# sonbui25/Multimodal-Aspect-Category-Sentiment-Analysis

Measured on AMD Instinct MI355X. Metric: train samples/sec (fwd+bwd+step) FCMF seq128x36ROI, higher is better.
Workload: dtype bf16; 1 GPU; FCMF-base fine-tune step, BASELINE configs[1]: batch 64 reviews x 6 aspects per GPU, seq 128, 7 images x (49 patches + 36 ROIs), precomputed ResNet-152 features, dropout 0.1, clip 1.0 + 4-group AdamW + linear schedule; global_batch=64, per_gpu_batch=64, seq_len=128, parallelism=dp1, sample_unit=1 review = 6 aspect forwards

## Files before the change

multimodal-aspect-category-sentiment-analysis_amd/csrc/attn_mfma.hip:

```cpp
#include "attn_tiles.h"
#include <cstdlib>


template <int NKT>
__device__ __forceinline__ void attn_mfma_fwd_tile(const AttnMfmaParams& P, int g, int h, int q0, int lane, const bf16x8 (&qf)[2][2],
                                                   const char* Ks, const char* Vs, const float* mask_lds = nullptr) {
  constexpr int NKF = 8 * NKT;
  const float* mrow = P.mask ? P.mask + (int64_t)g * P.Tk : nullptr;
  int nvalid = P.Tk;
  if (mask_lds || mrow) {
    int last = -1;
#pragma unroll
    for (int i = 0; i < 2 * NKT; ++i) {
      const int key = 64 * i + lane;
      const bool live = key < P.Tk && (mask_lds ? mask_lds[key] : mrow[key]) > -1e30f;
      const unsigned long long b = __ballot(live);
      if (b) last = 64 * i + 63 - __builtin_clzll(b);
    }
    nvalid = last >= 0 ? last + 1 : P.Tk;
  }
  f32x4 sc[NKF][2];
#pragma unroll
  for (int kf = 0; kf < NKF; ++kf)
#pragma unroll
    for (int f = 0; f < 2; ++f) sc[kf][f] = f32x4{0.f, 0.f, 0.f, 0.f};
#pragma unroll
  for (int s = 0; s < 2; ++s)
#pragma unroll
    for (int kf = 0; kf < NKF; ++kf) {
      if (16 * kf >= nvalid) continue;
      const bf16x8 ka = frag_row64(Ks, 16 * kf, s, lane);
#pragma unroll
      for (int f = 0; f < 2; ++f) sc[kf][f] = __builtin_amdgcn_mfma_f32_16x16x32_bf16(ka, qf[f][s], sc[kf][f], 0, 0, 0);
    }
  const float inv_keep = P.p > 0.f ? 1.0f / (1.0f - P.p) : 1.0f;
#pragma unroll
  for (int f = 0; f < 2; ++f) {
    const int q = q0 + 16 * f + (lane & 15);
    float m = -INFINITY;
#pragma unroll
    for (int kf = 0; kf < NKF; ++kf) {
      if (16 * kf >= nvalid) continue;
#pragma unroll
      for (int r = 0; r < 4; ++r) {
        const int key = 16 * kf + 4 * (lane >> 4) + r;
        float s = -INFINITY;
        if (key < P.Tk) s = sc[kf][f][r] * P.scale + (mask_lds ? mask_lds[key] : (mrow ? mrow[key] : 0.f));
        sc[kf][f][r] = s;
        m = fmaxf(m, s);
      }
    }
    m = fmaxf(m, __shfl_xor(m, 16, 64));
    m = fmaxf(m, __shfl_xor(m, 32, 64));
    float sum = 0.f;
#pragma unroll
    for (int kf = 0; kf < NKF; ++kf) {
      if (16 * kf >= nvalid) continue;
#pragma unroll
      for (int r = 0; r < 4; ++r) {
        const float e = __expf(sc[kf][f][r] - m);
        sc[kf][f][r] = e;
        sum += e;
      }
    }
    sum += __shfl_xor(sum, 16, 64);
    sum += __shfl_xor(sum, 32, 64);
    const float inv = 1.0f / sum;
    if (q < P.Tq && (lane >> 4) == 0 && P.lse) P.lse[((int64_t)g * P.heads + h) * P.Tq + q] = m + __logf(sum);
#pragma unroll
    for (int kf = 0; kf < NKF; ++kf) {
      if (16 * kf >= nvalid) continue;
      float dm[4] = {1.f, 1.f, 1.f, 1.f};
      if (P.p > 0.f)
        dropout_mult4(P.seed, ((uint64_t)g * P.heads + h) * P.Tq * P.Tk + (__umul24((unsigned)q, (unsigned)P.Tk) + (unsigned)(16 * kf + 4 * (lane >> 4))),
                      P.p, inv_keep, dm);
#pragma unroll
      for (int r = 0; r < 4; ++r) sc[kf][f][r] = sc[kf][f][r] * inv * dm[r];
    }
  }
  f32x4 oc[4][2];
#pragma unroll
  for (int df = 0; df < 4; ++df)
#pragma unroll
    for (int f = 0; f < 2; ++f) oc[df][f] = f32x4{0.f, 0.f, 0.f, 0.f};
#pragma unroll
  for (int s = 0; s < 4 * NKT; ++s) {
    if (32 * s >= nvalid) continue;
    bf16x8 pb[2];
#pragma unroll
    for (int f = 0; f < 2; ++f)
#pragma unroll
      for (int r = 0; r < 4; ++r) { pb[f][r] = (bf16_t)sc[2 * s][f][r]; pb[f][4 + r] = (bf16_t)sc[2 * s + 1][f][r]; }
#pragma unroll
    for (int df = 0; df < 4; ++df) {
      const bf16x8 va = frag_tr64p(Vs, 16 * df, s, lane);
#pragma unroll
      for (int f = 0; f < 2; ++f) oc[df][f] = __builtin_amdgcn_mfma_f32_16x16x32_bf16(va, pb[f], oc[df][f], 0, 0, 0);
    }
  }
#pragma unroll
  for (int f = 0; f < 2; ++f) {
    const int q = q0 + 16 * f + (lane & 15);
    if (q < P.Tq) {
      bf16_t* orow = P.out + ((int64_t)g * P.Tq + q) * P.ldo + h * AD + 4 * (lane >> 4);
#pragma unroll
      for (int df = 0; df < 4; ++df) store4(orow + 16 * df, oc[df][f]);
    }
  }
}

template <int NKT>
__device__ __forceinline__ void attn_mfma_fwd_body(const AttnMfmaParams& P) {
  extern __shared__ __attribute__((aligned(16))) char smem[];
  char* Ks = smem;
  char* Vs = smem + NKT * TILE_B;
  const int tid = threadIdx.x, lane = tid & 63, w = tid >> 6;
  const int g = blockIdx.x / P.heads, h = blockIdx.x % P.heads;
  const int q0 = blockIdx.y * AT + w * 32;
  const bf16_t* kbase_p = P.k + (int64_t)g * P.Tk * P.ldk + h * AD;
  const bf16_t* vbase_p = P.v + (int64_t)g * P.Tk * P.ldk + h * AD;
  const TileRegs kt = load_tile(kbase_p, P.ldk, P.Tk, tid);
  const TileRegs vt = load_tile(vbase_p, P.ldk, P.Tk, tid);
  bf16x8 qf[2][2];
  load_q_frags(P, g, h, q0, lane, qf);
  store_tile<false>(Ks, kt, tid);
  store_tile<true>(Vs, vt, tid);
  if constexpr (NKT == 2) {
    const TileRegs kt2 = load_tile(kbase_p + (int64_t)AT * P.ldk, P.ldk, P.Tk - AT, tid);
    const TileRegs vt2 = load_tile(vbase_p + (int64_t)AT * P.ldk, P.ldk, P.Tk - AT, tid);
    store_tile<false>(Ks + TILE_B, kt2, tid);
    store_tile<true>(Vs + TILE_B, vt2, tid);
  }
  __syncthreads();
  attn_mfma_fwd_tile<NKT>(P, g, h, q0, lane, qf, Ks, Vs);
}

__global__ __launch_bounds__(256, 2) void attn_mfma_fwd_persist_kernel(AttnMfmaParams P, int ntiles, int qtiles) {
  extern __shared__ __attribute__((aligned(16))) char smem[];
  const int tid = threadIdx.x, lane = tid & 63, w = tid >> 6;
  auto where = [&](int tile, int& g, int& h, int& q0) {
    const int gh = tile / qtiles;
    g = gh / P.heads; h = gh - g * P.heads; q0 = (tile - gh * qtiles) * AT + w * 32;
  };
  constexpr int BUF = 2 * TILE_B + 512;
  int tile = blockIdx.x;
  if (tile >= ntiles) return;
  int g, h, q0;
  where(tile, g, h, q0);
  bf16x8 qf[2][2];
  auto mask_of = [&](int gg) { return (P.mask && tid < P.Tk) ? P.mask[(int64_t)gg * P.Tk + tid] : 0.f; };
  {
    const TileRegs kt = load_tile(P.k + (int64_t)g * P.Tk * P.ldk + h * AD, P.ldk, P.Tk, tid);
    const TileRegs vt = load_tile(P.v + (int64_t)g * P.Tk * P.ldk + h * AD, P.ldk, P.Tk, tid);
    const float mv = mask_of(g);
    load_q_frags(P, g, h, q0, lane, qf);
    store_tile<false>(smem, kt, tid);
    store_tile<true>(smem + TILE_B, vt, tid);
    if (tid < AT) reinterpret_cast<float*>(smem + 2 * TILE_B)[tid] = mv;
  }
  __syncthreads();
  int cur = 0;
  for (;;) {
    const int nxt = tile + gridDim.x;
    const bool more = nxt < ntiles;
    int g2 = g, h2 = h, q2 = q0;
    TileRegs kt, vt;
    bf16x8 qn[2][2];
    float mv = 0.f;
    if (more) {
      where(nxt, g2, h2, q2);
      kt = load_tile(P.k + (int64_t)g2 * P.Tk * P.ldk + h2 * AD, P.ldk, P.Tk, tid);
      vt = load_tile(P.v + (int64_t)g2 * P.Tk * P.ldk + h2 * AD, P.ldk, P.Tk, tid);
      mv = mask_of(g2);
      load_q_frags(P, g2, h2, q2, lane, qn);
    }
    const char* buf = smem + cur * BUF;
    attn_mfma_fwd_tile<1>(P, g, h, q0, lane, qf, buf, buf + TILE_B, reinterpret_cast<const float*>(buf + 2 * TILE_B));
    if (!more) break;
    cur ^= 1;
    store_tile<false>(smem + cur * BUF, kt, tid);
    store_tile<true>(smem + cur * BUF + TILE_B, vt, tid);
    if (tid < AT) reinterpret_cast<float*>(smem + cur * BUF + 2 * TILE_B)[tid] = mv;
#pragma unroll
    for (int f = 0; f < 2; ++f)
#pragma unroll
      for (int s2 = 0; s2 < 2; ++s2) qf[f][s2] = qn[f][s2];
    g = g2; h = h2; q0 = q2; tile = nxt;
    __syncthreads();
  }
}

__global__ __launch_bounds__(256, 3) void attn_mfma_fwd_kernel(AttnMfmaParams P) { attn_mfma_fwd_body<1>(P); }
__global__ __launch_bounds__(256, 2) void attn_mfma_fwd256_kernel(AttnMfmaParams P) { attn_mfma_fwd_body<2>(P); }

template <int NQT, int NKT>
__device__ __forceinline__ void attn_mfma_bwd_body(const AttnMfmaParams& P) {
  extern __shared__ __attribute__((aligned(16))) char smem[];
  char* Qs = smem;
  char* dOs = Qs + NQT * TILE_B;
  char* Ks = dOs + NQT * TILE_B;
  char* Vs = Ks + NKT * TILE_B;
  char* PdT = Vs + NKT * TILE_B;
  char* dST = PdT + TILE_B / 2;
  const int tid = threadIdx.x, lane = tid & 63, w = tid >> 6;
  const int g = blockIdx.x / P.heads, h = blockIdx.x % P.heads;
  const int64_t qbase = (int64_t)g * P.Tq, kbase = (int64_t)g * P.Tk;
  float dl4[NQT][2][4], lse4[NQT][2][4];
  {
    TileRegs tq[NQT], td[NQT];
#pragma unroll
    for (int qt = 0; qt < NQT; ++qt) {
      tq[qt] = load_tile(P.q + (qbase + qt * AT) * P.ldq + h * AD, P.ldq, P.Tq - qt * AT, tid);
      td[qt] = load_tile(P.dout + (qbase + qt * AT) * P.ldo + h * AD, P.ldo, P.Tq - qt * AT, tid);
    }
    TileRegs tk = load_tile(P.k + kbase * P.ldk + h * AD, P.ldk, P.Tk, tid);
    TileRegs tv = load_tile(P.v + kbase * P.ldk + h * AD, P.ldk, P.Tk, tid);
#pragma unroll
    for (int qt = 0; qt < NQT; ++qt) {
      const int q = qt * AT + 32 * w + (lane >> 1), half = lane & 1;
      float sd = 0.f;
      if (q < P.Tq) {
        const bf16_t* a = P.dout + (qbase + q) * P.ldo + h * AD + 32 * half;
        const bf16_t* b = P.o + (qbase + q) * P.ldo + h * AD + 32 * half;
#pragma unroll
        for (int i = 0; i < 4; ++i) {
          const bf16x8 x = *reinterpret_cast<const bf16x8*>(a + 8 * i);
          const bf16x8 y = *reinterpret_cast<const bf16x8*>(b + 8 * i);
#pragma unroll
          for (int j = 0; j < 8; ++j) sd += (float)x[j] * (float)y[j];
        }
      }
      sd += __shfl_xor(sd, 1, 64);
#pragma unroll
      for (int f = 0; f < 2; ++f)
#pragma unroll
        for (int r = 0; r < 4; ++r) {
          const int ql = 16 * f + 4 * (lane >> 4) + r;
          dl4[qt][f][r] = __shfl(sd, 2 * ql, 64);
          const int q2 = qt * AT + 32 * w + ql;
          lse4[qt][f][r] = q2 < P.Tq ? P.lse[((int64_t)g * P.heads + h) * P.Tq + q2] : 0.f;
        }
    }
#pragma unroll
    for (int qt = 0; qt < NQT; ++qt) {
      store_tile<false>(Qs + qt * TILE_B, tq[qt], tid);
      store_tile<false>(dOs + qt * TILE_B, td[qt], tid);
    }
    store_tile<false>(Ks, tk, tid);
    store_tile<false>(Vs, tv, tid);
    if constexpr (NKT == 2) {
      tk = load_tile(P.k + (kbase + AT) * P.ldk + h * AD, P.ldk, P.Tk - AT, tid);
      tv = load_tile(P.v + (kbase + AT) * P.ldk + h * AD, P.ldk, P.Tk - AT, tid);
      store_tile<false>(Ks + TILE_B, tk, tid);
      store_tile<false>(Vs + TILE_B, tv, tid);
    }
  }
  __syncthreads();

  const float inv_keep = P.p > 0.f ? 1.0f / (1.0f - P.p) : 1.0f;
  const uint64_t drop_base = ((uint64_t)g * P.heads + h) * P.Tq * P.Tk;
  const float* mrow = P.mask ? P.mask + kbase : nullptr;
  float score_scale = P.scale;
  bf16x8 qa[NQT][2][2], da[NQT][2][2], oT[NQT][4], qT[NQT][4];
  f32x4 aQ[NQT][4][2];
#pragma unroll
  for (int qt = 0; qt < NQT; ++qt) {
#pragma unroll
    for (int f = 0; f < 2; ++f)
#pragma unroll
      for (int s = 0; s < 2; ++s) {
        qa[qt][f][s] = frag_row64(Qs + qt * TILE_B, 32 * w + 16 * f, s, lane);
        da[qt][f][s] = frag_row64(dOs + qt * TILE_B, 32 * w + 16 * f, s, lane);
      }
#pragma unroll
    for (int s = 0; s < 4; ++s) {
      oT[qt][s] = frag_tr64(dOs + qt * TILE_B, 16 * w, s, lane);
      qT[qt][s] = frag_tr64(Qs + qt * TILE_B, 16 * w, s, lane);
    }
#pragma unroll
    for (int df = 0; df < 4; ++df)
#pragma unroll
      for (int f = 0; f < 2; ++f) aQ[qt][df][f] = f32x4{0.f, 0.f, 0.f, 0.f};
  }

  const int nchunks_all = (P.Tk + 31) >> 5;
  int nvalid = P.Tk;
  if (mrow) {
    int last = -1;
#pragma unroll
    for (int i = 0; i < 2 * NKT; ++i) {
      const int key = 64 * i + lane;
      const bool live = key < P.Tk && mrow[key] > -1e30f;
      const unsigned long long b = __ballot(live);
      if (b) last = 64 * i + 63 - __builtin_clzll(b);
    }
    nvalid = last >= 0 ? last + 1 : P.Tk;
    if (last < 0) {
      mrow = nullptr;
      score_scale = 0.f;
      const float ltk = __logf((float)P.Tk);
#pragma unroll
      for (int qt = 0; qt < NQT; ++qt)
#pragma unroll
        for (int f = 0; f < 2; ++f)
#pragma unroll
          for (int r = 0; r < 4; ++r) lse4[qt][f][r] = ltk;
    }
  }
  const int nchunks = (nvalid + 31) >> 5;
  const uint64_t pair_base = drop_base >> 1;
  const uint32_t pb_lo = (uint32_t)pair_base, pb_hi = (uint32_t)(pair_base >> 32);
  const bool share_hash = P.p > 0.f && (P.Tk & 1) == 0 && pb_lo <= 0xFFFF0000u;
  const uint32_t hash_k0 = (uint32_t)P.seed ^ ((pb_hi << 7) | (pb_hi >> 25)), hash_s1 = (uint32_t)(P.seed >> 32);
  const uint32_t drop_thr = dropout_threshold(P.p);
  const int odd = lane & 1;
  f32x4 cV = f32x4{0.f, 0.f, 0.f, 0.f}, cK = f32x4{0.f, 0.f, 0.f, 0.f};
  for (int c = 0; c < nchunks; ++c) {
    f32x4 aV[2], aK[2];
#pragma unroll
    for (int kf = 0; kf < 2; ++kf) { aV[kf] = f32x4{0.f, 0.f, 0.f, 0.f}; aK[kf] = f32x4{0.f, 0.f, 0.f, 0.f}; }
#pragma unroll
    for (int qt = 0; qt < NQT; ++qt) {
      f32x4 sS[2][2], sP[2][2];
#pragma unroll
      for (int k4 = 0; k4 < 2; ++k4)
#pragma unroll
        for (int f = 0; f < 2; ++f) { sS[k4][f] = f32x4{0.f, 0.f, 0.f, 0.f}; sP[k4][f] = f32x4{0.f, 0.f, 0.f, 0.f}; }
#pragma unroll
      for (int s = 0; s < 2; ++s)
#pragma unroll
        for (int k4 = 0; k4 < 2; ++k4) {
          const bf16x8 kb = frag_row64(Ks, 32 * c + 16 * k4, s, lane);
          const bf16x8 vb = frag_row64(Vs, 32 * c + 16 * k4, s, lane);
#pragma unroll
          for (int f = 0; f < 2; ++f) {
            sS[k4][f] = __builtin_amdgcn_mfma_f32_16x16x32_bf16(qa[qt][f][s], kb, sS[k4][f], 0, 0, 0);
            sP[k4][f] = __builtin_amdgcn_mfma_f32_16x16x32_bf16(da[qt][f][s], vb, sP[k4][f], 0, 0, 0);
          }
        }
#pragma unroll
      for (int k4 = 0; k4 < 2; ++k4) {
        const int kl = 16 * k4 + (lane & 15), key = 32 * c + kl;
        const float mk = (mrow && key < P.Tk) ? mrow[key] : 0.f;
#pragma unroll
        for (int f = 0; f < 2; ++f) {
          f32x4 pdv, dsv;
          float mult4[4] = {1.0f, 1.0f, 1.0f, 1.0f};
          if (share_hash) {
            const unsigned q0 = qt * AT + 32 * w + 16 * f + 4 * (lane >> 4);
            const uint32_t o0 = pb_lo + __umul24(q0 + 2 * odd, (unsigned)P.Tk >> 1) + ((unsigned)key >> 1);
            const uint32_t hA = fcmf_hash32_rounds(o0 ^ hash_k0, hash_s1);
            const uint32_t hB = fcmf_hash32_rounds((o0 + ((unsigned)P.Tk >> 1)) ^ hash_k0, hash_s1);
            const uint32_t nA = (uint32_t)__builtin_amdgcn_update_dpp(0, (int)hA, 0xB1, 0xf, 0xf, true);
            const uint32_t nB = (uint32_t)__builtin_amdgcn_update_dpp(0, (int)hB, 0xB1, 0xf, 0xf, true);
            const uint32_t hr[4] = {odd ? nA : hA, odd ? nB : hB, odd ? hA : nA, odd ? hB : nB};
#pragma unroll
            for (int r = 0; r < 4; ++r) mult4[r] = ((hr[r] >> (16 * odd)) & 0xFFFFu) >= drop_thr ? inv_keep : 0.f;
          }
#pragma unroll
          for (int r = 0; r < 4; ++r) {
            const int q = qt * AT + 32 * w + 16 * f + 4 * (lane >> 4) + r;
            float pr = 0.f, mult = mult4[r];
            if (key < P.Tk && q < P.Tq) pr = __expf(sS[k4][f][r] * score_scale + mk - lse4[qt][f][r]);
            if (P.p > 0.f && !share_hash) mult = dropout_mult(P.seed, drop_base + (__umul24((unsigned)q, (unsigned)P.Tk) + (unsigned)key), P.p, inv_keep);
            pdv[r] = pr * mult;
            dsv[r] = pr * (sP[k4][f][r] * mult - dl4[qt][f][r]);
          }
          const int ch = 4 * w + 2 * f + (lane >> 5);
          const int o = off128(kl, ch) + ((lane >> 4) & 1) * 8;
          store4(reinterpret_cast<bf16_t*>(PdT + o), pdv);
          store4(reinterpret_cast<bf16_t*>(dST + o), dsv);
        }
      }
      __syncthreads();
      {
        bf16x8 tb[2];
#pragma unroll
        for (int f = 0; f < 2; ++f) tb[f] = frag_tr128(dST, 32 * w + 16 * f, 0, lane);
#pragma unroll
        for (int df = 0; df < 4; ++df) {
          const bf16x8 ka2 = frag_tr64(Ks, 16 * df, c, lane);
#pragma unroll
          for (int f = 0; f < 2; ++f) aQ[qt][df][f] = __builtin_amdgcn_mfma_f32_16x16x32_bf16(ka2, tb[f], aQ[qt][df][f], 0, 0, 0);
        }
      }
#pragma unroll
      for (int s = 0; s < 4; ++s)
#pragma unroll
        for (int kf = 0; kf < 2; ++kf) {
          const bf16x8 pb = frag_row128(PdT, 16 * kf, s, lane);
          const bf16x8 sb = frag_row128(dST, 16 * kf, s, lane);
          aV[kf] = __builtin_amdgcn_mfma_f32_16x16x32_bf16(oT[qt][s], pb, aV[kf], 0, 0, 0);
          aK[kf] = __builtin_amdgcn_mfma_f32_16x16x32_bf16(qT[qt][s], sb, aK[kf], 0, 0, 0);
        }
      __syncthreads();
    }
    const int dcol = h * AD + 16 * w + 4 * (lane >> 4);
    cV += aV[0] + aV[1];
    cK += aK[0] + aK[1];
#pragma unroll
    for (int kf = 0; kf < 2; ++kf) {
      const int key = 32 * c + 16 * kf + (lane & 15);
      if (key < P.Tk) {
        store4(P.dv + (kbase + key) * P.ldk + dcol, aV[kf]);
        f32x4 t = aK[kf];
        t[0] *= P.scale; t[1] *= P.scale; t[2] *= P.scale; t[3] *= P.scale;
        store4(P.dk + (kbase + key) * P.ldk + dcol, t);
      }
    }
  }
  for (int c = nchunks; c < nchunks_all; ++c) {
    const int dcol = h * AD + 16 * w + 4 * (lane >> 4);
#pragma unroll
    for (int kf = 0; kf < 2; ++kf) {
      const int key = 32 * c + 16 * kf + (lane & 15);
      if (key < P.Tk) {
        store4(P.dv + (kbase + key) * P.ldk + dcol, f32x4{0.f, 0.f, 0.f, 0.f});
        store4(P.dk + (kbase + key) * P.ldk + dcol, f32x4{0.f, 0.f, 0.f, 0.f});
      }
    }
  }
#pragma unroll
  for (int qt = 0; qt < NQT; ++qt)
#pragma unroll
    for (int f = 0; f < 2; ++f) {
      const int x = qt * AT + 32 * w + 16 * f + (lane & 15);
      if (x < P.Tq) {
        const int dcol = h * AD + 4 * (lane >> 4);
#pragma unroll
        for (int df = 0; df < 4; ++df) {
          f32x4 t = aQ[qt][df][f];
          t[0] *= P.scale; t[1] *= P.scale; t[2] *= P.scale; t[3] *= P.scale;
          store4(P.dq + (qbase + x) * P.ldq + dcol + 16 * df, t);
        }
      }
    }
  if (P.colsum) {
    const int HD = P.heads * AD;
    float* row = P.colsum + (int64_t)g * 3 * HD + h * AD;
#pragma unroll
    for (int r = 0; r < 4; ++r) { cV[r] = row16_sum(cV[r]); cK[r] = row16_sum(cK[r]); }
    if ((lane & 15) == 0) {
      const int d0 = 16 * w + 4 * (lane >> 4);
#pragma unroll
      for (int r = 0; r < 4; ++r) { row[2 * HD + d0 + r] = cV[r]; row[HD + d0 + r] = cK[r] * P.scale; }
    }
    float* red = reinterpret_cast<float*>(PdT);
#pragma unroll
    for (int df = 0; df < 4; ++df) {
      f32x4 t = f32x4{0.f, 0.f, 0.f, 0.f};
#pragma unroll
      for (int qt = 0; qt < NQT; ++qt)
#pragma unroll
        for (int f = 0; f < 2; ++f) t += aQ[qt][df][f];
#pragma unroll
      for (int r = 0; r < 4; ++r) t[r] = row16_sum(t[r]);
      if ((lane & 15) == 0) {
#pragma unroll
        for (int r = 0; r < 4; ++r) red[w * 64 + 16 * df + 4 * (lane >> 4) + r] = t[r];
      }
    }
    __syncthreads();
    if (tid < 64) row[tid] = (red[tid] + red[64 + tid] + red[128 + tid] + red[192 + tid]) * P.scale;
  }
}

__global__ __launch_bounds__(256, 2) void attn_mfma_bwd_kernel(AttnMfmaParams P) { attn_mfma_bwd_body<1, 1>(P); }
__global__ __launch_bounds__(256, 1) void attn_mfma_bwd256_kernel(AttnMfmaParams P) { attn_mfma_bwd_body<2, 2>(P); }

static bool al16(const void* p) { return (reinterpret_cast<uintptr_t>(p) & 15) == 0; }

extern "C" int fcmf_attn_mfma_fwd(const void* q, const void* k, const void* v, const float* mask, void* out, float* lse,
                                  int G, int heads, int Tq, int Tk, int64_t ldq, int64_t ldk, int64_t ldo, float scale,
                                  float dropout_p, uint64_t seed, void* stream) {
  if (!q || !k || !v || !out || G <= 0 || heads <= 0 || Tq <= 0 || Tk <= 0) return FCMF_ERR_ARG;
  if (Tk > 2 * AT || ldq % 8 || ldk % 8 || ldo % 4 || !al16(q) || !al16(k) || !al16(v) || !al16(out)) return FCMF_ERR_UNSUPPORTED;
  AttnMfmaParams P{};
  P.q = (const bf16_t*)q; P.k = (const bf16_t*)k; P.v = (const bf16_t*)v; P.mask = mask; P.out = (bf16_t*)out; P.lse = lse;
  P.G = G; P.heads = heads; P.Tq = Tq; P.Tk = Tk; P.ldq = ldq; P.ldk = ldk; P.ldo = ldo;
  P.scale = scale; P.p = dropout_p; P.seed = seed;
  const dim3 grid(G * heads, (Tq + AT - 1) / AT);
  if (Tk > AT) {
    const int smem = 4 * TILE_B;
    static bool attr2 = false;
    return fcmf_launch_flagged(&attr2, attn_mfma_fwd256_kernel, grid, dim3(256), smem, reinterpret_cast<hipStream_t>(stream), P);
  }
  const int ntiles = (int)(grid.x * grid.y);
  static const bool no_persist = getenv("FCMF_ATTN_NO_PERSIST") != nullptr;
  if (ntiles >= 4 * 512 && !no_persist) {
    const int smem = 2 * (2 * TILE_B + 512);
    static bool attr3 = false;
    return fcmf_launch_flagged(&attr3, attn_mfma_fwd_persist_kernel, dim3(512), dim3(256), smem, reinterpret_cast<hipStream_t>(stream), P, ntiles, (int)grid.y);
  }
  const int smem = 2 * TILE_B;
  static bool attr = false;
  return fcmf_launch_flagged(&attr, attn_mfma_fwd_kernel, grid, dim3(256), smem, reinterpret_cast<hipStream_t>(stream), P);
}

extern "C" int fcmf_attn_mfma_bwd(const void* q, const void* k, const void* v, const float* mask, const void* out,
                                  const void* dout, const float* lse, void* dq, void* dk, void* dv, int G, int heads,
                                  int Tq, int Tk, int64_t ldq, int64_t ldk, int64_t ldo, float scale, float dropout_p,
                                  uint64_t seed, float* colsum, void* stream) {
  if (!q || !k || !v || !out || !dout || !lse || !dq || !dk || !dv || G <= 0 || heads <= 0 || Tq <= 0 || Tk <= 0) return FCMF_ERR_ARG;
  if (Tk > 2 * AT || Tq > 2 * AT || ldq % 8 || ldk % 8 || ldo % 8 || !al16(q) || !al16(k) || !al16(v) || !al16(out) || !al16(dout) ||
      !al16(dq) || !al16(dk) || !al16(dv))
    return FCMF_ERR_UNSUPPORTED;
  AttnMfmaParams P{};
  P.q = (const bf16_t*)q; P.k = (const bf16_t*)k; P.v = (const bf16_t*)v; P.mask = mask; P.o = (const bf16_t*)out;
  P.dout = (const bf16_t*)dout; P.lse = const_cast<float*>(lse); P.dq = (bf16_t*)dq; P.dk = (bf16_t*)dk; P.dv = (bf16_t*)dv;
  P.G = G; P.heads = heads; P.Tq = Tq; P.Tk = Tk; P.ldq = ldq; P.ldk = ldk; P.ldo = ldo;
  P.scale = scale; P.p = dropout_p; P.seed = seed; P.colsum = colsum;
  if (Tk > AT || Tq > AT) {
    const int smem = 9 * TILE_B;
    static bool attr2 = false;
    return fcmf_launch_flagged(&attr2, attn_mfma_bwd256_kernel, dim3(G * heads), dim3(256), smem, reinterpret_cast<hipStream_t>(stream), P);
  }
  const int smem = 5 * TILE_B;
  static bool attr = false;
  return fcmf_launch_flagged(&attr, attn_mfma_bwd_kernel, dim3(G * heads), dim3(256), smem, reinterpret_cast<hipStream_t>(stream), P);
}
```

multimodal-aspect-category-sentiment-analysis_amd/csrc/attn_tiles.h:

```cpp
#pragma once
#include "common.h"

constexpr int AD = 64;
constexpr int AT = 128;
constexpr int TILE_B = AT * AD * 2;

__device__ __forceinline__ int vkey(int r) { return ((r >> 1) & 1) | (((r >> 3) & 1) << 1); }
__device__ __forceinline__ int off64(int r, int c8) { return r * 128 + ((((c8 >> 1) ^ vkey(r))) << 5) + ((c8 & 1) << 4); }
__device__ __forceinline__ int key16(int r) { return ((r & 7) << 1) ^ (((r >> 3) & 1) * 9); }
__device__ __forceinline__ int off128(int r, int ch) { return r * 256 + ((ch ^ key16(r)) << 4); }
__device__ __forceinline__ int offp(int r, int ch) { return r * 256 + ((ch ^ (r & 15)) << 4); }

__device__ __forceinline__ int off64p(int r, int c8) { return r * 128 + ((((c8 >> 1) ^ ((r >> 1) & 3))) << 5) + ((c8 & 1) << 4); }

typedef bf16x4 __attribute__((address_space(3))) * lds_v4_t;

__device__ __forceinline__ void stage_tile(char* lds, const bf16_t* __restrict__ src, int64_t ld, int rows, int tid) {
#pragma unroll
  for (int i = 0; i < 4; ++i) {
    const int c = tid + 256 * i, r = c >> 3, c8 = c & 7;
    uint4 v = make_uint4(0, 0, 0, 0);
    if (r < rows) v = *reinterpret_cast<const uint4*>(src + (int64_t)r * ld + c8 * 8);
    *reinterpret_cast<uint4*>(lds + off64(r, c8)) = v;
  }
}
__device__ __forceinline__ void stage_tile_p(char* lds, const bf16_t* __restrict__ src, int64_t ld, int rows, int tid) {
#pragma unroll
  for (int i = 0; i < 4; ++i) {
    const int c = tid + 256 * i, r = c >> 3, c8 = c & 7;
    uint4 v = make_uint4(0, 0, 0, 0);
    if (r < rows) v = *reinterpret_cast<const uint4*>(src + (int64_t)r * ld + c8 * 8);
    *reinterpret_cast<uint4*>(lds + off64p(r, c8)) = v;
  }
}
__device__ __forceinline__ bf16x8 frag_tr64p(const char* lds, int c0, int s, int lane) {
  const int g4 = lane >> 4, i16 = lane & 15, q4 = i16 >> 2, p = i16 & 3;
  const int r = 32 * s + 4 * g4 + q4, c8 = (c0 >> 3) + (p >> 1);
  bf16x4 lo = __builtin_amdgcn_ds_read_tr16_b64_v4bf16((lds_v4_t)(lds + off64p(r, c8) + (p & 1) * 8));
  bf16x4 hi = __builtin_amdgcn_ds_read_tr16_b64_v4bf16((lds_v4_t)(lds + off64p(r + 16, c8) + (p & 1) * 8));
  bf16x8 o;
  o[0] = lo[0]; o[1] = lo[1]; o[2] = lo[2]; o[3] = lo[3]; o[4] = hi[0]; o[5] = hi[1]; o[6] = hi[2]; o[7] = hi[3];
  return o;
}
struct TileRegs { uint4 v[4]; };
__device__ __forceinline__ TileRegs load_tile(const bf16_t* __restrict__ src, int64_t ld, int rows, int tid) {
  TileRegs t;
#pragma unroll
  for (int i = 0; i < 4; ++i) {
    const int c = tid + 256 * i, r = c >> 3, c8 = c & 7;
    t.v[i] = make_uint4(0, 0, 0, 0);
    if (r < rows) t.v[i] = *reinterpret_cast<const uint4*>(src + (int64_t)r * ld + c8 * 8);
  }
  return t;
}
template <bool PERMUTED>
__device__ __forceinline__ void store_tile(char* lds, const TileRegs& t, int tid) {
#pragma unroll
  for (int i = 0; i < 4; ++i) {
    const int c = tid + 256 * i, r = c >> 3, c8 = c & 7;
    *reinterpret_cast<uint4*>(lds + (PERMUTED ? off64p(r, c8) : off64(r, c8))) = t.v[i];
  }
}
__device__ __forceinline__ bf16x8 frag_row64(const char* lds, int x0, int s, int lane) {
  return *reinterpret_cast<const bf16x8*>(lds + off64(x0 + (lane & 15), 4 * s + (lane >> 4)));
}
__device__ __forceinline__ bf16x8 frag_tr64(const char* lds, int c0, int s, int lane) {
  const int g4 = lane >> 4, i16 = lane & 15, q4 = i16 >> 2, p = i16 & 3;
  const int r = 32 * s + 8 * g4 + q4, c8 = (c0 >> 3) + (p >> 1);
  bf16x4 lo = __builtin_amdgcn_ds_read_tr16_b64_v4bf16((lds_v4_t)(lds + off64(r, c8) + (p & 1) * 8));
  bf16x4 hi = __builtin_amdgcn_ds_read_tr16_b64_v4bf16((lds_v4_t)(lds + off64(r + 4, c8) + (p & 1) * 8));
  bf16x8 o;
  o[0] = lo[0]; o[1] = lo[1]; o[2] = lo[2]; o[3] = lo[3]; o[4] = hi[0]; o[5] = hi[1]; o[6] = hi[2]; o[7] = hi[3];
  return o;
}
__device__ __forceinline__ bf16x8 frag_row128(const char* lds, int x0, int s, int lane) {
  return *reinterpret_cast<const bf16x8*>(lds + off128(x0 + (lane & 15), 4 * s + (lane >> 4)));
}
__device__ __forceinline__ bf16x8 frag_tr128(const char* lds, int c0, int s, int lane) {
  const int g4 = lane >> 4, i16 = lane & 15, q4 = i16 >> 2, p = i16 & 3;
  const int r = 32 * s + 8 * g4 + q4, ch = (c0 >> 3) + (p >> 1);
  bf16x4 lo = __builtin_amdgcn_ds_read_tr16_b64_v4bf16((lds_v4_t)(lds + off128(r, ch) + (p & 1) * 8));
  bf16x4 hi = __builtin_amdgcn_ds_read_tr16_b64_v4bf16((lds_v4_t)(lds + off128(r + 4, ch) + (p & 1) * 8));
  bf16x8 o;
  o[0] = lo[0]; o[1] = lo[1]; o[2] = lo[2]; o[3] = lo[3]; o[4] = hi[0]; o[5] = hi[1]; o[6] = hi[2]; o[7] = hi[3];
  return o;
}
__device__ __forceinline__ void store4(bf16_t* p, f32x4 v) {
  bf16x4 o;
  o[0] = (bf16_t)v[0]; o[1] = (bf16_t)v[1]; o[2] = (bf16_t)v[2]; o[3] = (bf16_t)v[3];
  *reinterpret_cast<bf16x4*>(p) = o;
}

__device__ __forceinline__ float row16_sum(float x) {
#define FCMF_ROR_ADD(n) x += __builtin_bit_cast(float, __builtin_amdgcn_update_dpp(0, __builtin_bit_cast(int, x), 0x120 + (n), 0xf, 0xf, true))
  FCMF_ROR_ADD(8); FCMF_ROR_ADD(4); FCMF_ROR_ADD(2); FCMF_ROR_ADD(1);
#undef FCMF_ROR_ADD
  return x;
}

struct AttnMfmaParams {
  const bf16_t *q, *k, *v, *o, *dout;
  const float* mask;
  bf16_t *out, *dq, *dk, *dv;
  float* lse;
  float* colsum;
  int G, heads, Tq, Tk;
  int64_t ldq, ldk, ldo;
  float scale, p;
  uint64_t seed;
};

__device__ __forceinline__ void load_q_frags(const AttnMfmaParams& P, int g, int h, int q0, int lane, bf16x8 (&qf)[2][2]) {
#pragma unroll
  for (int f = 0; f < 2; ++f)
#pragma unroll
    for (int s = 0; s < 2; ++s) {
      const int row = q0 + 16 * f + (lane & 15);
      uint4 v = make_uint4(0, 0, 0, 0);
      if (row < P.Tq) v = *reinterpret_cast<const uint4*>(P.q + ((int64_t)g * P.Tq + row) * P.ldq + h * AD + 32 * s + 8 * (lane >> 4));
      qf[f][s] = *reinterpret_cast<bf16x8*>(&v);
    }
}
```

Measured before the change: 1773 samples/s.

## Restructure attention kernels with clamped loads, LDS-staged dK/dV/dQ stores, deferred stores

Global loads in the forward persistent and backward attention kernels become unconditional clamped loads with register-side zeroing, so the loads are no longer predicated. In the persistent forward kernel, output and LSE stores are deferred until after the next tile is staged to LDS, overlapping the stores with the compute. In the backward kernel, the mask is preloaded into registers, the D=rowsum(dO*O) dot product reads dO from LDS, and dK/dV/dQ are staged through swizzled LDS so they are written as coalesced 16-byte rows. The LDS staging reuses the K/V buffers after use and adds some synchronisation and complexity.

```diff
diff --git a/multimodal-aspect-category-sentiment-analysis_amd/csrc/attn_mfma.hip b/multimodal-aspect-category-sentiment-analysis_amd/csrc/attn_mfma.hip
--- a/multimodal-aspect-category-sentiment-analysis_amd/csrc/attn_mfma.hip
+++ b/multimodal-aspect-category-sentiment-analysis_amd/csrc/attn_mfma.hip
@@ -2,9 +2,10 @@
 #include <cstdlib>
 
 
-template <int NKT>
-__device__ __forceinline__ void attn_mfma_fwd_tile(const AttnMfmaParams& P, int g, int h, int q0, int lane, const bf16x8 (&qf)[2][2],
-                                                   const char* Ks, const char* Vs, const float* mask_lds = nullptr) {
+template <int NKT, bool LSE_LATE>
+__device__ __forceinline__ void attn_mfma_fwd_tile_compute(const AttnMfmaParams& P, int g, int h, int q0, int lane, const bf16x8 (&qf)[2][2],
+                                                           const char* Ks, const char* Vs, const float* mask_lds, f32x4 (&oc)[4][2],
+                                                           float (&lv)[2]) {
   constexpr int NKF = 8 * NKT;
   const float* mrow = P.mask ? P.mask + (int64_t)g * P.Tk : nullptr;
   int nvalid = P.Tk;
@@ -66,7 +67,8 @@
     sum += __shfl_xor(sum, 16, 64);
     sum += __shfl_xor(sum, 32, 64);
     const float inv = 1.0f / sum;
-    if (q < P.Tq && (lane >> 4) == 0 && P.lse) P.lse[((int64_t)g * P.heads + h) * P.Tq + q] = m + __logf(sum);
+    lv[f] = m + __logf(sum);
+    if (!LSE_LATE && q < P.Tq && (lane >> 4) == 0 && P.lse) P.lse[((int64_t)g * P.heads + h) * P.Tq + q] = lv[f];
 #pragma unroll
     for (int kf = 0; kf < NKF; ++kf) {
       if (16 * kf >= nvalid) continue;
@@ -78,7 +80,6 @@
       for (int r = 0; r < 4; ++r) sc[kf][f][r] = sc[kf][f][r] * inv * dm[r];
     }
   }
-  f32x4 oc[4][2];
 #pragma unroll
   for (int df = 0; df < 4; ++df)
 #pragma unroll
@@ -98,15 +99,28 @@
       for (int f = 0; f < 2; ++f) oc[df][f] = __builtin_amdgcn_mfma_f32_16x16x32_bf16(va, pb[f], oc[df][f], 0, 0, 0);
     }
   }
+}
+template <bool LSE_LATE>
+__device__ __forceinline__ void attn_mfma_fwd_tile_store(const AttnMfmaParams& P, int g, int h, int q0, int lane, const f32x4 (&oc)[4][2],
+                                                         const float (&lv)[2]) {
 #pragma unroll
   for (int f = 0; f < 2; ++f) {
     const int q = q0 + 16 * f + (lane & 15);
     if (q < P.Tq) {
+      if (LSE_LATE && (lane >> 4) == 0 && P.lse) P.lse[((int64_t)g * P.heads + h) * P.Tq + q] = lv[f];
       bf16_t* orow = P.out + ((int64_t)g * P.Tq + q) * P.ldo + h * AD + 4 * (lane >> 4);
 #pragma unroll
       for (int df = 0; df < 4; ++df) store4(orow + 16 * df, oc[df][f]);
     }
   }
+}
+template <int NKT>
+__device__ __forceinline__ void attn_mfma_fwd_tile(const AttnMfmaParams& P, int g, int h, int q0, int lane, const bf16x8 (&qf)[2][2],
+                                                   const char* Ks, const char* Vs, const float* mask_lds = nullptr) {
+  f32x4 oc[4][2];
+  float lv[2];
+  attn_mfma_fwd_tile_compute<NKT, false>(P, g, h, q0, lane, qf, Ks, Vs, mask_lds, oc, lv);
+  attn_mfma_fwd_tile_store<false>(P, g, h, q0, lane, oc, lv);
 }
 
 template <int NKT>
@@ -148,36 +162,36 @@
   int g, h, q0;
   where(tile, g, h, q0);
   bf16x8 qf[2][2];
-  auto mask_of = [&](int gg) { return (P.mask && tid < P.Tk) ? P.mask[(int64_t)gg * P.Tk + tid] : 0.f; };
+  auto mask_of = [&](int gg) { return P.mask ? P.mask[(int64_t)gg * P.Tk + min(tid, P.Tk - 1)] : 0.f; };
   {
-    const TileRegs kt = load_tile(P.k + (int64_t)g * P.Tk * P.ldk + h * AD, P.ldk, P.Tk, tid);
-    const TileRegs vt = load_tile(P.v + (int64_t)g * P.Tk * P.ldk + h * AD, P.ldk, P.Tk, tid);
+    TileRegs kt = load_tile_clamped(P.k + (int64_t)g * P.Tk * P.ldk + h * AD, P.ldk, P.Tk, tid);
+    TileRegs vt = load_tile_clamped(P.v + (int64_t)g * P.Tk * P.ldk + h * AD, P.ldk, P.Tk, tid);
     const float mv = mask_of(g);
-    load_q_frags(P, g, h, q0, lane, qf);
+    load_q_frags_clamped(P, g, h, q0, lane, qf);
+    zero_tail(kt, P.Tk, tid);
+    zero_tail(vt, P.Tk, tid);
+    zero_q_tail(P, q0, lane, qf);
     store_tile<false>(smem, kt, tid);
     store_tile<true>(smem + TILE_B, vt, tid);
     if (tid < AT) reinterpret_cast<float*>(smem + 2 * TILE_B)[tid] = mv;
   }
   __syncthreads();
   int cur = 0;
-  for (;;) {
-    const int nxt = tile + gridDim.x;
-    const bool more = nxt < ntiles;
-    int g2 = g, h2 = h, q2 = q0;
-    TileRegs kt, vt;
+  for (int nxt = tile + gridDim.x; nxt < ntiles; nxt += gridDim.x) {
+    int g2, h2, q2;
     bf16x8 qn[2][2];
-    float mv = 0.f;
-    if (more) {
-      where(nxt, g2, h2, q2);
-      kt = load_tile(P.k + (int64_t)g2 * P.Tk * P.ldk + h2 * AD, P.ldk, P.Tk, tid);
-      vt = load_tile(P.v + (int64_t)g2 * P.Tk * P.ldk + h2 * AD, P.ldk, P.Tk, tid);
-      mv = mask_of(g2);
-      load_q_frags(P, g2, h2, q2, lane, qn);
-    }
+    where(nxt, g2, h2, q2);
+    TileRegs kt = load_tile_clamped(P.k + (int64_t)g2 * P.Tk * P.ldk + h2 * AD, P.ldk, P.Tk, tid);
+    TileRegs vt = load_tile_clamped(P.v + (int64_t)g2 * P.Tk * P.ldk + h2 * AD, P.ldk, P.Tk, tid);
+    const float mv = mask_of(g2);
+    load_q_frags_clamped(P, g2, h2, q2, lane, qn);
     const char* buf = smem + cur * BUF;
-    attn_mfma_fwd_tile<1>(P, g, h, q0, lane, qf, buf, buf + TILE_B, reinterpret_cast<const float*>(buf + 2 * TILE_B));
-    if (!more) break;
+    f32x4 oc[4][2];
+    float lv[2];
+    attn_mfma_fwd_tile_compute<1, true>(P, g, h, q0, lane, qf, buf, buf + TILE_B, reinterpret_cast<const float*>(buf + 2 * TILE_B), oc, lv);
     cur ^= 1;
+    zero_tail(kt, P.Tk, tid);
+    zero_tail(vt, P.Tk, tid);
     store_tile<false>(smem + cur * BUF, kt, tid);
     store_tile<true>(smem + cur * BUF + TILE_B, vt, tid);
     if (tid < AT) reinterpret_cast<float*>(smem + cur * BUF + 2 * TILE_B)[tid] = mv;
@@ -185,9 +199,14 @@
     for (int f = 0; f < 2; ++f)
 #pragma unroll
       for (int s2 = 0; s2 < 2; ++s2) qf[f][s2] = qn[f][s2];
-    g = g2; h = h2; q0 = q2; tile = nxt;
+    zero_q_tail(P, q2, lane, qf);
+    asm volatile("" : "+v"(qf[0][0]), "+v"(qf[0][1]), "+v"(qf[1][0]), "+v"(qf[1][1]) : : "memory");
+    attn_mfma_fwd_tile_store<true>(P, g, h, q0, lane, oc, lv);
+    g = g2; h = h2; q0 = q2;
     __syncthreads();
   }
+  const char* buf = smem + cur * BUF;
+  attn_mfma_fwd_tile<1>(P, g, h, q0, lane, qf, buf, buf + TILE_B, reinterpret_cast<const float*>(buf + 2 * TILE_B));
 }
 
 __global__ __launch_bounds__(256, 3) void attn_mfma_fwd_kernel(AttnMfmaParams P) { attn_mfma_fwd_body<1>(P); }
@@ -206,60 +225,78 @@
   const int g = blockIdx.x / P.heads, h = blockIdx.x % P.heads;
   const int64_t qbase = (int64_t)g * P.Tq, kbase = (int64_t)g * P.Tk;
   float dl4[NQT][2][4], lse4[NQT][2][4];
+  float mreg[2 * NKT];
   {
-    TileRegs tq[NQT], td[NQT];
+    TileRegs tq[NQT], td[NQT], tk[NKT], tv[NKT];
+    uint4 og[NQT][4];
 #pragma unroll
     for (int qt = 0; qt < NQT; ++qt) {
-      tq[qt] = load_tile(P.q + (qbase + qt * AT) * P.ldq + h * AD, P.ldq, P.Tq - qt * AT, tid);
-      td[qt] = load_tile(P.dout + (qbase + qt * AT) * P.ldo + h * AD, P.ldo, P.Tq - qt * AT, tid);
-    }
-    TileRegs tk = load_tile(P.k + kbase * P.ldk + h * AD, P.ldk, P.Tk, tid);
-    TileRegs tv = load_tile(P.v + kbase * P.ldk + h * AD, P.ldk, P.Tk, tid);
+      tq[qt] = load_tile_clamped(P.q + (qbase + qt * AT) * P.ldq + h * AD, P.ldq, P.Tq - qt * AT, tid);
+      td[qt] = load_tile_clamped(P.dout + (qbase + qt * AT) * P.ldo + h * AD, P.ldo, P.Tq - qt * AT, tid);
+    }
+#pragma unroll
+    for (int kt = 0; kt < NKT; ++kt) {
+      tk[kt] = load_tile_clamped(P.k + (kbase + kt * AT) * P.ldk + h * AD, P.ldk, P.Tk - kt * AT, tid);
+      tv[kt] = load_tile_clamped(P.v + (kbase + kt * AT) * P.ldk + h * AD, P.ldk, P.Tk - kt * AT, tid);
+    }
 #pragma unroll
     for (int qt = 0; qt < NQT; ++qt) {
-      const int q = qt * AT + 32 * w + (lane >> 1), half = lane & 1;
-      float sd = 0.f;
-      if (q < P.Tq) {
-        const bf16_t* a = P.dout + (qbase + q) * P.ldo + h * AD + 32 * half;
-        const bf16_t* b = P.o + (qbase + q) * P.ldo + h * AD + 32 * half;
-#pragma unroll
-        for (int i = 0; i < 4; ++i) {
-          const bf16x8 x = *reinterpret_cast<const bf16x8*>(a + 8 * i);
-          const bf16x8 y = *reinterpret_cast<const bf16x8*>(b + 8 * i);
-#pragma unroll
-          for (int j = 0; j < 8; ++j) sd += (float)x[j] * (float)y[j];
+      const int q = min(qt * AT + 32 * w + (lane >> 1), P.Tq - 1);
+      const bf16_t* b = P.o + (qbase + q) * P.ldo + h * AD + 32 * (lane & 1);
+#pragma unroll
+      for (int i = 0; i < 4; ++i) og[qt][i] = *reinterpret_cast<const uint4*>(b + 8 * i);
+#pragma unroll
+      for (int f = 0; f < 2; ++f)
+#pragma unroll
+        for (int r = 0; r < 4; ++r) {
+          const int q2 = qt * AT + 32 * w + 16 * f + 4 * (lane >> 4) + r;
+          lse4[qt][f][r] = P.lse[((int64_t)g * P.heads + h) * P.Tq + min(q2, P.Tq - 1)];
         }
-      }
-      sd += __shfl_xor(sd, 1, 64);
-#pragma unroll
-      for (int f = 0; f < 2; ++f)
-#pragma unroll
-        for (int r = 0; r < 4; ++r) {
-          const int ql = 16 * f + 4 * (lane >> 4) + r;
-          dl4[qt][f][r] = __shfl(sd, 2 * ql, 64);
-          const int q2 = qt * AT + 32 * w + ql;
-          lse4[qt][f][r] = q2 < P.Tq ? P.lse[((int64_t)g * P.heads + h) * P.Tq + q2] : 0.f;
-        }
-    }
+    }
+#pragma unroll
+    for (int i = 0; i < 2 * NKT; ++i) mreg[i] = P.mask ? P.mask[kbase + min(64 * i + lane, P.Tk - 1)] : 0.f;
 #pragma unroll
     for (int qt = 0; qt < NQT; ++qt) {
+      zero_tail(tq[qt], P.Tq - qt * AT, tid);
+      zero_tail(td[qt], P.Tq - qt * AT, tid);
       store_tile<false>(Qs + qt * TILE_B, tq[qt], tid);
       store_tile<false>(dOs + qt * TILE_B, td[qt], tid);
     }
-    store_tile<false>(Ks, tk, tid);
-    store_tile<false>(Vs, tv, tid);
-    if constexpr (NKT == 2) {
-      tk = load_tile(P.k + (kbase + AT) * P.ldk + h * AD, P.ldk, P.Tk - AT, tid);
-      tv = load_tile(P.v + (kbase + AT) * P.ldk + h * AD, P.ldk, P.Tk - AT, tid);
-      store_tile<false>(Ks + TILE_B, tk, tid);
-      store_tile<false>(Vs + TILE_B, tv, tid);
-    }
-  }
-  __syncthreads();
+#pragma unroll
+    for (int kt = 0; kt < NKT; ++kt) {
+      zero_tail(tk[kt], P.Tk - kt * AT, tid);
+      zero_tail(tv[kt], P.Tk - kt * AT, tid);
+      store_tile<false>(Ks + kt * TILE_B, tk[kt], tid);
+      store_tile<false>(Vs + kt * TILE_B, tv[kt], tid);
+    }
+    __syncthreads();
+#pragma unroll
+    for (int qt = 0; qt < NQT; ++qt) {
+      const int ql = 32 * w + (lane >> 1), half = lane & 1;
+      float sd = 0.f;
+#pragma unroll
+      for (int i = 0; i < 4; ++i) {
+        const bf16x8 x = *reinterpret_cast<const bf16x8*>(dOs + qt * TILE_B + off64(ql, 4 * half + i));
+        const bf16x8 y = *reinterpret_cast<const bf16x8*>(&og[qt][i]);
+#pragma unroll
+        for (int j = 0; j < 8; ++j) sd += (float)x[j] * (float)y[j];
+      }
+      if (qt * AT + ql >= P.Tq) sd = 0.f;
+      sd += __shfl_xor(sd, 1, 64);
+#pragma unroll
+      for (int f = 0; f < 2; ++f)
+#pragma unroll
+        for (int r = 0; r < 4; ++r) {
+          const int qr = 16 * f + 4 * (lane >> 4) + r;
+          dl4[qt][f][r] = __shfl(sd, 2 * qr, 64);
+          if (qt * AT + 32 * w + qr >= P.Tq) lse4[qt][f][r] = 0.f;
+        }
+    }
+  }
 
   const float inv_keep = P.p > 0.f ? 1.0f / (1.0f - P.p) : 1.0f;
   const uint64_t drop_base = ((uint64_t)g * P.heads + h) * P.Tq * P.Tk;
-  const float* mrow = P.mask ? P.mask + kbase : nullptr;
+  bool masked = P.mask != nullptr;
   float score_scale = P.scale;
   bf16x8 qa[NQT][2][2], da[NQT][2][2], oT[NQT][4], qT[NQT][4];
   f32x4 aQ[NQT][4][2];
@@ -285,18 +322,19 @@
 
   const int nchunks_all = (P.Tk + 31) >> 5;
   int nvalid = P.Tk;
-  if (mrow) {
+  if (masked) {
     int last = -1;
 #pragma unroll
     for (int i = 0; i < 2 * NKT; ++i) {
       const int key = 64 * i + lane;
-      const bool live = key < P.Tk && mrow[key] > -1e30f;
+      const bool live = key < P.Tk && mreg[i] > -1e30f;
+      if (key >= P.Tk) mreg[i] = 0.f;
       const unsigned long long b = __ballot(live);
       if (b) last = 64 * i + 63 - __builtin_clzll(b);
     }
     nvalid = last >= 0 ? last + 1 : P.Tk;
     if (last < 0) {
-      mrow = nullptr;
+      masked = false;
       score_scale = 0.f;
       const float ltk = __logf((float)P.Tk);
 #pragma unroll
@@ -315,10 +353,27 @@
   const uint32_t drop_thr = dropout_threshold(P.p);
   const int odd = lane & 1;
   f32x4 cV = f32x4{0.f, 0.f, 0.f, 0.f}, cK = f32x4{0.f, 0.f, 0.f, 0.f};
+  auto flush_dkv = [&](int cc) {
+    const int r = tid >> 3, ch = tid & 7, key = 32 * cc + r;
+    const int o = cc * (TILE_B / 4) + r * 128 + ((ch ^ ((r >> 1) & 7)) << 4);
+    const uint4 dvv = *reinterpret_cast<const uint4*>(Vs + o), dkk = *reinterpret_cast<const uint4*>(Ks + o);
+    if (key < P.Tk) {
+      *reinterpret_cast<uint4*>(P.dv + (kbase + key) * P.ldk + h * AD + 8 * ch) = dvv;
+      *reinterpret_cast<uint4*>(P.dk + (kbase + key) * P.ldk + h * AD + 8 * ch) = dkk;
+    }
+  };
   for (int c = 0; c < nchunks; ++c) {
     f32x4 aV[2], aK[2];
 #pragma unroll
     for (int kf = 0; kf < 2; ++kf) { aV[kf] = f32x4{0.f, 0.f, 0.f, 0.f}; aK[kf] = f32x4{0.f, 0.f, 0.f, 0.f}; }
+    float mk2[2] = {0.f, 0.f};
+    if (masked) {
+      float mc = mreg[0];
+#pragma unroll
+      for (int i = 1; i < 2 * NKT; ++i) mc = (c >> 1) == i ? mreg[i] : mc;
+#pragma unroll
+      for (int k4 = 0; k4 < 2; ++k4) mk2[k4] = __shfl(mc, 32 * (c & 1) + 16 * k4 + (lane & 15), 64);
+    }
 #pragma unroll
     for (int qt = 0; qt < NQT; ++qt) {
       f32x4 sS[2][2], sP[2][2];
@@ -341,7 +396,7 @@
 #pragma unroll
       for (int k4 = 0; k4 < 2; ++k4) {
         const int kl = 16 * k4 + (lane & 15), key = 32 * c + kl;
-        const float mk = (mrow && key < P.Tk) ? mrow[key] : 0.f;
+        const float mk = mk2[k4];
 #pragma unroll
         for (int f = 0; f < 2; ++f) {
           f32x4 pdv, dsv;
@@ -373,6 +428,7 @@
         }
       }
       __syncthreads();
+      if (qt == 0 && c > 0) flush_dkv(c - 1);
       {
         bf16x8 tb[2];
 #pragma unroll
@@ -395,46 +451,47 @@
         }
       __syncthreads();
     }
-    const int dcol = h * AD + 16 * w + 4 * (lane >> 4);
     cV += aV[0] + aV[1];
     cK += aK[0] + aK[1];
 #pragma unroll
     for (int kf = 0; kf < 2; ++kf) {
-      const int key = 32 * c + 16 * kf + (lane & 15);
-      if (key < P.Tk) {
-        store4(P.dv + (kbase + key) * P.ldk + dcol, aV[kf]);
-        f32x4 t = aK[kf];
+      const int kl = 16 * kf + (lane & 15);
+      const int o = c * (TILE_B / 4) + kl * 128 + (((2 * w + (lane >> 5)) ^ ((kl >> 1) & 7)) << 4) + ((lane >> 4) & 1) * 8;
+      store4(reinterpret_cast<bf16_t*>(Vs + o), aV[kf]);
+      f32x4 t = aK[kf];
+      t[0] *= P.scale; t[1] *= P.scale; t[2] *= P.scale; t[3] *= P.scale;
+      store4(reinterpret_cast<bf16_t*>(Ks + o), t);
+    }
+  }
+  __syncthreads();
+  flush_dkv(nchunks - 1);
+  for (int c = nchunks; c < nchunks_all; ++c) {
+    const int key = 32 * c + (tid >> 3);
+    if (key < P.Tk) {
+      *reinterpret_cast<uint4*>(P.dv + (kbase + key) * P.ldk + h * AD + 8 * (tid & 7)) = make_uint4(0, 0, 0, 0);
+      *reinterpret_cast<uint4*>(P.dk + (kbase + key) * P.ldk + h * AD + 8 * (tid & 7)) = make_uint4(0, 0, 0, 0);
+    }
+  }
+  char* stg = PdT + w * (TILE_B / 4);
+#pragma unroll
+  for (int qt = 0; qt < NQT; ++qt) {
+#pragma unroll
+    for (int f = 0; f < 2; ++f) {
+      const int ql = 16 * f + (lane & 15);
+#pragma unroll
+      for (int df = 0; df < 4; ++df) {
+        f32x4 t = aQ[qt][df][f];
         t[0] *= P.scale; t[1] *= P.scale; t[2] *= P.scale; t[3] *= P.scale;
-        store4(P.dk + (kbase + key) * P.ldk + dcol, t);
-      }
-    }
-  }
-  for (int c = nchunks; c < nchunks_all; ++c) {
-    const int dcol = h * AD + 16 * w + 4 * (lane >> 4);
-#pragma unroll
-    for (int kf = 0; kf < 2; ++kf) {
-      const int key = 32 * c + 16 * kf + (lane & 15);
-      if (key < P.Tk) {
-        store4(P.dv + (kbase + key) * P.ldk + dcol, f32x4{0.f, 0.f, 0.f, 0.f});
-        store4(P.dk + (kbase + key) * P.ldk + dcol, f32x4{0.f, 0.f, 0.f, 0.f});
-      }
-    }
-  }
-#pragma unroll
-  for (int qt = 0; qt < NQT; ++qt)
-#pragma unroll
-    for (int f = 0; f < 2; ++f) {
-      const int x = qt * AT + 32 * w + 16 * f + (lane & 15);
-      if (x < P.Tq) {
-        const int dcol = h * AD + 4 * (lane >> 4);
-#pragma unroll
-        for (int df = 0; df < 4; ++df) {
-          f32x4 t = aQ[qt][df][f];
-          t[0] *= P.scale; t[1] *= P.scale; t[2] *= P.scale; t[3] *= P.scale;
-          store4(P.dq + (qbase + x) * P.ldq + dcol + 16 * df, t);
-        }
-      }
-    }
+        store4(reinterpret_cast<bf16_t*>(stg + ql * 128 + (((2 * df + (lane >> 5)) ^ ((ql >> 1) & 7)) << 4) + ((lane >> 4) & 1) * 8), t);
+      }
+    }
+#pragma unroll
+    for (int i = 0; i < 4; ++i) {
+      const int ql = 8 * i + (lane >> 3), ch = lane & 7, x = qt * AT + 32 * w + ql;
+      const uint4 v = *reinterpret_cast<const uint4*>(stg + ql * 128 + ((ch ^ ((ql >> 1) & 7)) << 4));
+      if (x < P.Tq) *reinterpret_cast<uint4*>(P.dq + (qbase + x) * P.ldq + h * AD + 8 * ch) = v;
+    }
+  }
   if (P.colsum) {
     const int HD = P.heads * AD;
     float* row = P.colsum + (int64_t)g * 3 * HD + h * AD;
@@ -445,6 +502,7 @@
 #pragma unroll
       for (int r = 0; r < 4; ++r) { row[2 * HD + d0 + r] = cV[r]; row[HD + d0 + r] = cK[r] * P.scale; }
     }
+    constexpr int RW = TILE_B / 4 / 4;
     float* red = reinterpret_cast<float*>(PdT);
 #pragma unroll
     for (int df = 0; df < 4; ++df) {
@@ -457,11 +515,11 @@
       for (int r = 0; r < 4; ++r) t[r] = row16_sum(t[r]);
       if ((lane & 15) == 0) {
 #pragma unroll
-        for (int r = 0; r < 4; ++r) red[w * 64 + 16 * df + 4 * (lane >> 4) + r] = t[r];
+        for (int r = 0; r < 4; ++r) red[w * RW + 16 * df + 4 * (lane >> 4) + r] = t[r];
       }
     }
     __syncthreads();
-    if (tid < 64) row[tid] = (red[tid] + red[64 + tid] + red[128 + tid] + red[192 + tid]) * P.scale;
+    if (tid < 64) row[tid] = (red[tid] + red[RW + tid] + red[2 * RW + tid] + red[3 * RW + tid]) * P.scale;
   }
 }
 
diff --git a/multimodal-aspect-category-sentiment-analysis_amd/csrc/attn_tiles.h b/multimodal-aspect-category-sentiment-analysis_amd/csrc/attn_tiles.h
--- a/multimodal-aspect-category-sentiment-analysis_amd/csrc/attn_tiles.h
+++ b/multimodal-aspect-category-sentiment-analysis_amd/csrc/attn_tiles.h
@@ -52,6 +52,20 @@
     if (r < rows) t.v[i] = *reinterpret_cast<const uint4*>(src + (int64_t)r * ld + c8 * 8);
   }
   return t;
+}
+__device__ __forceinline__ TileRegs load_tile_clamped(const bf16_t* __restrict__ src, int64_t ld, int rows, int tid) {
+  TileRegs t;
+#pragma unroll
+  for (int i = 0; i < 4; ++i) {
+    const int c = tid + 256 * i, r = c >> 3, c8 = c & 7;
+    t.v[i] = *reinterpret_cast<const uint4*>(src + (int64_t)min(r, rows - 1) * ld + c8 * 8);
+  }
+  return t;
+}
+__device__ __forceinline__ void zero_tail(TileRegs& t, int rows, int tid) {
+#pragma unroll
+  for (int i = 0; i < 4; ++i)
+    if (((tid + 256 * i) >> 3) >= rows) t.v[i] = make_uint4(0, 0, 0, 0);
 }
 template <bool PERMUTED>
 __device__ __forceinline__ void store_tile(char* lds, const TileRegs& t, int tid) {
@@ -121,3 +135,23 @@
       qf[f][s] = *reinterpret_cast<bf16x8*>(&v);
     }
 }
+__device__ __forceinline__ void load_q_frags_clamped(const AttnMfmaParams& P, int g, int h, int q0, int lane, bf16x8 (&qf)[2][2]) {
+#pragma unroll
+  for (int f = 0; f < 2; ++f)
+#pragma unroll
+    for (int s = 0; s < 2; ++s) {
+      const int row = min(q0 + 16 * f + (lane & 15), P.Tq - 1);
+      const uint4 v = *reinterpret_cast<const uint4*>(P.q + ((int64_t)g * P.Tq + row) * P.ldq + h * AD + 32 * s + 8 * (lane >> 4));
+      qf[f][s] = *reinterpret_cast<const bf16x8*>(&v);
+    }
+}
+__device__ __forceinline__ void zero_q_tail(const AttnMfmaParams& P, int q0, int lane, bf16x8 (&qf)[2][2]) {
+#pragma unroll
+  for (int f = 0; f < 2; ++f)
+    if (q0 + 16 * f + (lane & 15) >= P.Tq) {
+#pragma unroll
+      for (int s = 0; s < 2; ++s)
+#pragma unroll
+        for (int j = 0; j < 8; ++j) qf[f][s][j] = (bf16_t)0.f;
+    }
+}
```

Measured after the change: 1800 samples/s, median of 6. 1.02x the previous value.
